# MoonLab-YH/AOD_MEH_HUA

Hardware: AMD Instinct MI355X
Metric: images/sec train+HUA-score, RetinaNet-R50 VOC 512^2 (higher is better)
Workload: dtype bf16x3

## Files before the change

### aod_meh_hua_amd/_C.py

```python
import ctypes as C
import os

import torch

_HERE = os.path.dirname(os.path.abspath(__file__))
LIB_PATH = os.environ.get('AOD_HIP_LIB') or os.path.join(_HERE, 'lib', 'libaodhip.so')


class AodHipError(RuntimeError):
    pass


if not os.path.exists(LIB_PATH):
    raise ImportError(f'{LIB_PATH} is missing: run `python -m aod_meh_hua_amd.build` (hipcc, gfx950). '
                      'There is no CPU fallback for the MEH/HUA hot path.')
lib = C.CDLL(LIB_PATH)


class ConvSeg(C.Structure):
    _fields_ = [('B', C.c_int32), ('H', C.c_int32), ('W', C.c_int32), ('OH', C.c_int32), ('OW', C.c_int32),
                ('src_row0', C.c_int64), ('dst_row0', C.c_int64)]


class ConvDesc(C.Structure):
# ... 77 lines not shown
    'aod_meh_loss_levels_bwd': (C.c_int, [P, P, P, I32, P, P, P, I32, I32, I32, P]),
    'aod_softmax_rowmax': (C.c_int, [P, I32, I64, I32, F32, P, P, I32, P]),
    'aod_topk_stable': (C.c_int, [P, I32, I64, I32, P, I64, P]),
    'aod_pre_nms_levels': (C.c_int, [I32, P, P, P, P, P, P, I32, I32, F32, I32, I32, P, P, P, P, F32, P, P, P, P, P, P, P, I64, P]),
    'aod_gather_decode': (C.c_int, [P, P, P, P, P, I32, I64, I32, I32, I64, P, P, P, P, F32, P, P, P, P, I64, I64, I64, I32, P]),
    'aod_nms_ws_bytes': (SZ, [I32, I32, I32]),
    'aod_multiclass_nms': (C.c_int, [P, P, I32, I32, I32, F32, F32, I32, P, P, P, P, P, P]),
    'aod_hua_ws_bytes': (SZ, [I32, I32]),
    'aod_hua_score': (C.c_int, [P, P, P, P, P, P, P, P, P, I32, I32, I32, I32, I32, F32, F32, F32, I32, U64, P, I32, I32, I32, P, P, I32, P, P, P]),
    'aod_maxpool_fwd': (C.c_int, [P, P, I32, I32, I32, I32, I32, I32, I32, I32, I32, P]),
    'aod_maxpool_bwd': (C.c_int, [P, P, P, I32, I32, I32, I32, I32, I32, I32, I32, I32, P]),
    'aod_l2norm_fwd': (C.c_int, [P, P, P, I64, I32, F32, P]),
    'aod_l2norm_bwd': (C.c_int, [P, P, P, P, P, I64, I32, F32, P]),
    'aod_ssd_loss_fwd': (C.c_int, [P, P, P, P, P, P, I32, I32, I32, I32, I32, F32, P, P, P, P]),
    'aod_ssd_loss_bwd': (C.c_int, [P, P, P, P, P, P, P, P, I32, I32, I32, I32, F32, P, P, P, P, P, P]),
    'aod_synth_normal_images': (C.c_int, [P, I32, I64, U64, P, P]),
    'aod_image_xform': (C.c_int, [P, P, I32, I32, I32, P, P]),
    'aod_x3_split': (C.c_int, [P, P, I64, I32, P]),
    'aod_x3_merge': (C.c_int, [P, P, I64, I32, P]),
    'aod_x3_add': (C.c_int, [P, P, P, I64, P]),
    'aod_x3_nchw_f32_to_s2d': (C.c_int, [P, P, I32, I32, I32, I32, P]),
    'aod_x3_maxpool3x3s2': (C.c_int, [P, P, I32, I32, I32, I32, P]),
    'aod_x3_upsample2x_add_to': (C.c_int, [P, P, P, I32, I32, I32, I32, I32, I32, P]),
    'aod_x3_upsample2x_add_bwd_set': (C.c_int, [P, P, I32, I32, I32, I32, I32, I32, P]),
    'aod_x3_act_bwd': (C.c_int, [P, P, P, P, I64, I32, I32, P]),
    'aod_x3_pad_cast_colsum': (C.c_int, [P, P, P, P, I64, I32, P]),
    'aod_x3_nchw_f32_to_nhwc': (C.c_int, [P, P, I32, I32, I32, I32, P]),
    'aod_x3_maxpool_fwd': (C.c_int, [P, P, I32, I32, I32, I32, I32, I32, I32, I32, I32, P]),
    'aod_x3_maxpool_bwd': (C.c_int, [P, P, P, I32, I32, I32, I32, I32, I32, I32, I32, I32, P]),
    'aod_x3_l2norm_fwd': (C.c_int, [P, P, P, I64, I32, F32, P]),
    'aod_x3_l2norm_bwd': (C.c_int, [P, P, P, P, P, I64, I32, F32, P]),
    'aod_sgd_multi': (C.c_int, [P, P, P, P, I32, F32, P, F32, F32, I32, F32, P]),
    'aod_sgd_multi_clipped': (C.c_int, [P, P, P, P, I32, F32, P, F32, F32, I32, F32, P, P]),
    'aod_grad_norm_multi': (C.c_int, [P, P, I32, F32, F32, I32, P, I64, P, P]),
}
for _n, (_r, _a) in _SIGS.items():
    if hasattr(lib, _n):
        getattr(lib, _n).restype = _r
        getattr(lib, _n).argtypes = _a
lib.aod_last_error.restype = C.c_char_p


def ptr(t):
    if t is None:
        return None
    if not t.is_cuda:
        raise AodHipError('aod_meh_hua_amd ops need tensors on the MI355X (cuda:N); got a CPU tensor. There is no CPU fallback.')
    return C.c_void_p(t.data_ptr())


def stream():
    return C.c_void_p(torch.cuda.current_stream().cuda_stream)


def check(rc, name='aod'):
    if rc != 0:
        raise AodHipError(f'{name} failed ({rc}): {lib.aod_last_error().decode()}')


def call(name, *args):
    check(getattr(lib, name)(*args), name)
```

### aod_meh_hua_amd/csrc/conv.hip

```cpp
#include "common.h"
#include "pointwise.h"
#include "conv_x3p.h"

struct ConvGroup { const bf16_t* x; const bf16_t* w; void* y; const float* pre_shift; const bf16_t* mask; float* colsum; };
struct ConvKParams {
  const bf16_t* x;
  const bf16_t* w;
  void* y;
  const float* pre_scale;
  const float* pre_shift;
  const bf16_t* res;
  const bf16_t* mask;
  const float* post_scale;
  bf16_t* zraw;
  float* colsum;
  int C, N, K, R, S, stride, pad, dil, transposed, relu, out_f32;
  int nseg, M;
  int tiles_m, tiles_n;
  int ksplit;
  float* ws;
  int perm;
  int ngroups;
  ConvGroup grp[4];
  int stagger;
// ... 2093 lines not shown
    __syncthreads();
  }
  if (a.wdot) {
    dot = wave_sum(dot);
    if ((threadIdx.x & 63) == 0) red[threadIdx.x >> 6] = dot;
    __syncthreads();
    if (threadIdx.x == 0) {
      float d = 0.f;
      for (int k = 0; k < UNP_T / 64; ++k) d += red[k];
      a.wdot[oo] = a.bn_s1 ? a.bn_invstd[oo] * (d - a.bn_mean[oo] * a.bn_s1[oo]) : d;
    }
  }
}
__global__ __launch_bounds__(UNP_T) void unpack_wgrad_slabs_kernel(const UnpackArgs a) {
  __shared__ float tile[UNP_CH * 9 + 1];
  __shared__ float red[UNP_T / 64];
  unpack_row(a, blockIdx.x, tile, red);
}
struct UnpackGroups { UnpackArgs g[WG_MAXG]; int blk0[WG_MAXG + 1]; };
__global__ __launch_bounds__(UNP_T) void unpack_wgrad_slabs_grouped_kernel(const UnpackGroups gp) {
  __shared__ float tile[UNP_CH * 9 + 1];
  __shared__ float red[UNP_T / 64];
  const int b = blockIdx.x;
  if (b < gp.blk0[1]) unpack_row(gp.g[0], b, tile, red);
  else if (b < gp.blk0[2]) unpack_row(gp.g[1], b - gp.blk0[1], tile, red);
  else if (b < gp.blk0[3]) unpack_row(gp.g[2], b - gp.blk0[2], tile, red);
  else unpack_row(gp.g[3], b - gp.blk0[3], tile, red);
}
struct PrepItem {
  const float* w; const float* gamma; const float* beta; const float* mean; const float* var;
  bf16_t* wf; bf16_t* wd; float* scale; float* shift; float* invstd;
  int O, I, RS, Ipad, Opad, blk0;
  float eps; int flags;
  long long pad2_[2];
};
constexpr int PREP_T = 32, PREP_RS = 9;
__global__ __launch_bounds__(256) void param_prep_kernel(const PrepItem* __restrict__ items, int nitems) {
  __shared__ float tile[PREP_RS][PREP_T][PREP_T + 1];
  int lo = 0, hi = nitems - 1;
  while (lo < hi) {
    const int mid = (lo + hi + 1) >> 1;
    if (items[mid].blk0 <= (int)blockIdx.x) lo = mid; else hi = mid - 1;
  }
  const PrepItem it = items[lo];
  const int lb = blockIdx.x - it.blk0;
  const int t = threadIdx.x;
  if (it.RS > PREP_RS) {
    const long long nf = (long long)it.O * it.RS * it.Ipad, nd = it.wd ? (long long)it.I * it.RS * it.Opad : 0;
    for (int u = 0; u < 8; ++u) {
      const long long i = (long long)lb * 2048 + u * 256 + t;
      const bool x3 = it.flags & 1;
      if (i < nf) {
        const int cp = i % it.Ipad; const long long r1 = i / it.Ipad; const int rs = r1 % it.RS; const int oo = r1 / it.RS;
        const int c = x3 ? ((cp >> 6) << 5) + (cp & 31) : cp;
        const float v = (c < it.I) ? it.w[((long long)oo * it.I + c) * it.RS + rs] : 0.f;
        const bf16_t h = (bf16_t)v;
        it.wf[i] = (x3 && (cp & 32)) ? (bf16_t)(v - (float)h) : h;
      }
      if (i < nd) {
        const int op = i % it.Opad; const long long r1 = i / it.Opad; const int rs = r1 % it.RS; const int c = r1 / it.RS;
        const int oo = x3 ? ((op >> 6) << 5) + (op & 31) : op;
        float v = 0.f;
        if (oo < it.O) { v = it.w[((long long)oo * it.I + c) * it.RS + rs]; if (it.gamma) v *= it.gamma[oo] * rsqrtf(it.var[oo] + it.eps); }
        const bf16_t h = (bf16_t)v;
        it.wd[i] = (x3 && (op & 32)) ? (bf16_t)(v - (float)h) : h;
      }
      if (it.gamma && i < it.O) {
        const float inv = rsqrtf(it.var[i] + it.eps), sc = it.gamma[i] * inv;
        it.invstd[i] = inv; it.scale[i] = sc; it.shift[i] = it.beta[i] - it.mean[i] * sc;
      }
    }
    return;
  }
  const bool x3 = it.flags & 1;
  const int Il = x3 ? it.Ipad >> 1 : it.Ipad, Ol = x3 ? it.Opad >> 1 : it.Opad;
  const int tiles_c = (Il + PREP_T - 1) / PREP_T;
  const int to = lb / tiles_c, tc = lb - to * tiles_c;
  const int o0 = to * PREP_T, c0 = tc * PREP_T;
  const int RS = it.RS;
  const int run = PREP_T * RS;
  const int pitch = run | 1;
  float* tl = &tile[0][0][0];
  const int cvalid = it.I - c0 < PREP_T ? it.I - c0 : PREP_T;
  {
    const int lim = cvalid * RS;
    const float* src0 = it.w + ((long long)o0 * it.I + c0) * RS;
    const long long ostride = (long long)it.I * RS;
    const bool al = ((((size_t)src0) | ((size_t)ostride * 4)) & 15) == 0;
    f32x4 v[PREP_RS];
    int ol[PREP_RS], idx[PREP_RS];
    const bool full = al && cvalid == PREP_T && o0 + PREP_T <= it.O;
#pragma unroll
    for (int k = 0; k < PREP_RS; ++k) {
      v[k] = (f32x4){0.f, 0.f, 0.f, 0.f};
      if (k < RS) {
        const int e = 4 * (t + k * 256);
        ol[k] = e / run; idx[k] = e - ol[k] * run;
        const float* sp = src0 + ol[k] * ostride + idx[k];
        if (full) v[k] = *reinterpret_cast<const f32x4*>(sp);
        else if (o0 + ol[k] < it.O) {
#pragma unroll
          for (int j = 0; j < 4; ++j) if (idx[k] + j < lim) v[k][j] = sp[j];
        }
      }
    }
#pragma unroll
    for (int k = 0; k < PREP_RS; ++k)
      if (k < RS) {
#pragma unroll
        for (int j = 0; j < 4; ++j) tl[ol[k] * pitch + idx[k] + j] = v[k][j];
      }
  }
  __syncthreads();
  for (int u = t; u < PREP_T * RS * 4; u += 256) {
    const int oct = u & 3, q = u >> 2, ol = q / RS, rs = q - ol * RS;
    const int o = o0 + ol, c = c0 + oct * 8;
    if (o < it.O && c < Il) {
// ... 12 lines not shown
    }
  }
  if (it.wd) {
    __shared__ float s_sc[PREP_T];
    if (t < PREP_T) {
      const int o = o0 + t;
      s_sc[t] = (it.gamma && o < it.O) ? it.gamma[o] * rsqrtf(it.var[o] + it.eps) : 1.f;
    }
    __syncthreads();
    for (int u = t; u < PREP_T * RS * 4; u += 256) {
      const int oct = u & 3, q = u >> 2, cl = q / RS, rs = q - cl * RS;
      const int c = c0 + cl, o = o0 + oct * 8;
      if (c < it.I && o < Ol) {
        bf16x8 v;
#pragma unroll
        for (int j = 0; j < 8; ++j) v[j] = (bf16_t)(tl[(oct * 8 + j) * pitch + cl * RS + rs] * s_sc[oct * 8 + j]);
        if (!x3) *reinterpret_cast<bf16x8*>(it.wd + ((long long)c * RS + rs) * it.Opad + o) = v;
        else {
          bf16x8 l;
#pragma unroll
          for (int j = 0; j < 8; ++j) l[j] = (bf16_t)(tl[(oct * 8 + j) * pitch + cl * RS + rs] * s_sc[oct * 8 + j] - (float)v[j]);
          bf16_t* d = it.wd + ((long long)c * RS + rs) * it.Opad + 2 * o0 + oct * 8;
          *reinterpret_cast<bf16x8*>(d) = v;
          *reinterpret_cast<bf16x8*>(d + 32) = l;
        }
      }
    }
  }
  if (it.gamma && tc == 0 && t < PREP_T && o0 + t < it.O) {
    const int o = o0 + t;
    const float inv = rsqrtf(it.var[o] + it.eps), sc = it.gamma[o] * inv;
    it.invstd[o] = inv; it.scale[o] = sc; it.shift[o] = it.beta[o] - it.mean[o] * sc;
  }
}
extern "C" int aod_param_prep(const void* items_dev, int nitems, int total_blocks, aod_stream_t stream) {
  AOD_CHECK_ARG(items_dev && nitems >= 0 && total_blocks >= 0, "param_prep: bad args");
  if (nitems == 0 || total_blocks == 0) return 0;
  hipLaunchKernelGGL(param_prep_kernel, dim3(total_blocks), dim3(256), 0, (hipStream_t)stream, (const PrepItem*)items_dev, nitems);
  AOD_LAUNCH_CHECK();
  return 0;
}
extern "C" int aod_param_prep_item_bytes(void) { return (int)sizeof(PrepItem); }

static inline int grid_for(long long n) { long long b = (n + 255) / 256; return (int)(b > 4096 ? 4096 : (b < 1 ? 1 : b)); }

extern "C" int aod_pack_weight_fwd(const float* w, void* o, int O, int I, int R, int S, int Ipad, aod_stream_t stream) {
  AOD_CHECK_ARG(w && o && Ipad >= I && Ipad % 8 == 0, "pack_weight_fwd: bad args");
  hipLaunchKernelGGL(pack_w_fwd_kernel, dim3(grid_for((long long)O * R * S * Ipad)), dim3(256), 0, (hipStream_t)stream, w, (bf16_t*)o, O, I, R * S, Ipad);
  AOD_LAUNCH_CHECK();
  return 0;
}
extern "C" int aod_pack_weight_dgrad(const float* w, void* o, int O, int I, int R, int S, int Opad, const float* scale, aod_stream_t stream) {
  AOD_CHECK_ARG(w && o && Opad >= O && Opad % 8 == 0, "pack_weight_dgrad: Opad must be a multiple of 8 and >= O");
  hipLaunchKernelGGL(pack_w_dgrad_kernel, dim3(grid_for((long long)Opad * R * S * I)), dim3(256), 0, (hipStream_t)stream, w, scale, (bf16_t*)o, O, I, R * S, Opad);
  AOD_LAUNCH_CHECK();
  return 0;
}
extern "C" int aod_unpack_wgrad_slabs(const float* dw_slabs, int nslabs, int64_t slab_stride, float* g, int O, int I, int R, int S, int Ipad,
                                      int accumulate, const float* scale, const float* w_oihw, float* wdot, const float* bn_s1,
                                      const float* bn_mean, const float* bn_invstd, aod_stream_t stream) {
  AOD_CHECK_ARG(dw_slabs && g && nslabs >= 1 && slab_stride > 0, "unpack_wgrad_slabs: null / empty");
  AOD_CHECK_ARG(R * S <= 16, "unpack_wgrad_slabs: at most 16 taps (larger filters take aod_unpack_wgrad)");
  AOD_CHECK_ARG(!wdot || w_oihw, "unpack_wgrad_slabs: wdot needs the weights");
  AOD_CHECK_ARG(!bn_s1 || (wdot && bn_mean && bn_invstd), "unpack_wgrad_slabs: BN mode needs wdot, mean and invstd");
  if (O == 0) return 0;
  UnpackArgs a;
// ... 46 lines not shown
```

### aod_meh_hua_amd/functional.py

```python
import torch
from torch.autograd import Function

from . import hipops as ho
from .hipops import Seg


def as_rows(x):
    B, C, H, W = x.shape
    xr = x.permute(0, 2, 3, 1)
    if not xr.is_contiguous():
        xr = xr.contiguous()
    return xr.view(B * H * W, C)


def as_nchw(rows, B, H, W):
    return rows.view(B, H, W, rows.shape[1]).permute(0, 3, 1, 2)


def multi_rows(tensors):
    rows = [as_rows(t) for t in tensors]
    if len(rows) == 1:
        t = tensors[0]
        return rows[0], [Seg(t.shape[0], t.shape[2], t.shape[3], 0)]
    rb = rows[0].shape[1] * rows[0].element_size()
# ... 11 lines not shown


def dense_segs(segs):
    out, r = [], 0
    for s in segs:
        out.append(Seg(s.B, s.H, s.W, r))
        r += s.rows
    return out


import ctypes as _C
import weakref as _weakref


class _PrepRec(_C.Structure):
    _fields_ = [('w', _C.c_void_p), ('gamma', _C.c_void_p), ('beta', _C.c_void_p), ('mean', _C.c_void_p), ('var', _C.c_void_p),
                ('wf', _C.c_void_p), ('wd', _C.c_void_p), ('scale', _C.c_void_p), ('shift', _C.c_void_p), ('invstd', _C.c_void_p),
                ('O', _C.c_int32), ('I', _C.c_int32), ('RS', _C.c_int32), ('Ipad', _C.c_int32), ('Opad', _C.c_int32), ('blk0', _C.c_int32),
                ('eps', _C.c_float), ('pad_', _C.c_int32), ('pad2_', _C.c_int64 * 2)]


class _FragRec(_C.Structure):
    _fields_ = [('src', _C.c_void_p), ('dst', _C.c_void_p), ('rows', _C.c_int32), ('K', _C.c_int32), ('blk0', _C.c_int32), ('pad_', _C.c_int32)]


class _PrepItem:
    __slots__ = ('srcs', 'ver', 'wf', 'wd', 'scale', 'shift', 'invstd', 'eps', 'dims', 'nblk', 'fragf', 'fragd', 'x3')


class ParamPrep:

    def __init__(self):
        self.items, self.order, self.table, self.dirty, self.tables = {}, [], None, True, {}
        self.stems = []

    def watch_stem(self, conv):
        self.stems = [r for r in self.stems if r() is not None and r() is not conv] + [_weakref.ref(conv)]

    def _versions(self, it):
        return tuple(-1 if t is None else t._version for t in (r() if r is not None else None for r in it.srcs))

    def get(self, w, bn, cin_pad, eps):
        it = self.items.get((id(w), ho.X3))
        if it is not None and it.srcs[0]() is not w:
            it = None
        if it is None:
            it = self._register(w, bn, cin_pad, eps)
        if it.ver != self._versions(it):
            self.refresh()
        return it

    def _register(self, w, bn, cin_pad, eps):
        O, I, R, S = w.shape
        dev = w.device
        it = _PrepItem()
        it.srcs = [_weakref.ref(w)] + [(_weakref.ref(t) if t is not None else None) for t in (bn if bn is not None else (None,) * 4)]
        it.x3 = ho.X3
        if it.x3:
            assert cin_pad == ho.xw(I), f'x3: input rows of {cin_pad} columns for a filter with {I} input channels'
            opad = ho.xw(O)
            it.wf = torch.empty(O, R, S, cin_pad, dtype=torch.bfloat16, device=dev)
            it.wd = torch.empty(I, R, S, opad, dtype=torch.bfloat16, device=dev) if I % 32 == 0 else None
        else:
            opad = (O + 7) // 8 * 8
            it.wf = torch.empty(O, R, S, cin_pad, dtype=torch.bfloat16, device=dev)
            it.wd = torch.empty(I, R, S, opad, dtype=torch.bfloat16, device=dev) if cin_pad == I else None
        if bn is not None:
            it.scale, it.shift, it.invstd = (torch.empty(O, dtype=torch.float32, device=dev) for _ in range(3))
        else:
            it.scale = it.shift = it.invstd = None
        it.eps, it.dims, it.ver = float(eps), (O, I, R * S, cin_pad, opad), None
        it.fragf = it.fragd = None
        if R * S <= 9 and it.x3:
            it.nblk = (opad // 64) * (cin_pad // 64)
        elif R * S <= 9:
            it.nblk = ((opad + 31) // 32) * ((cin_pad + 31) // 32)
        else:
            it.nblk = (max(O * R * S * cin_pad, I * R * S * opad if it.wd is not None else 0, O) + 2047) // 2048
        self.items[(id(w), it.x3)] = it
        self.dirty = True
        return it

    def frag(self, it, which):
        name = 'fragf' if which == 'f' else 'fragd'
        t = getattr(it, name)
        if t is None:
            src = it.wf if which == 'f' else it.wd
            rows = src.shape[0]
            assert rows % 256 == 0 and (src.numel() // rows) % 64 == 0, 'frag images need rows % 256 == 0 and K % 64 == 0'
            t = torch.empty(src.numel(), dtype=torch.bfloat16, device=src.device)
            setattr(it, name, t)
            self.tables, it.ver = {}, None
            self.refresh()
        return t

    def refresh_if_stale(self):
        for r in self.stems:
            conv = r()
            if conv is not None and not torch.cuda.is_current_stream_capturing():
                _stem_w4(conv)
        if any(it.x3 == ho.X3 and it.ver != self._versions(it) for it in self.items.values()):
            self.refresh()

    def refresh(self):
        assert not torch.cuda.is_current_stream_capturing(), \
            'parameter preparation inside a HIP-graph capture: call PREP.refresh_if_stale() before capturing / replaying'
        dead = [k for k, it in self.items.items() if it.srcs[0]() is None or any(r is not None and r() is None for r in it.srcs[1:])]
        for k in dead:
            del self.items[k]
            self.dirty = True
        if self.dirty:
            self.order = list(self.items.values())
            self.tables = {}
            self.dirty = False
        stale = tuple(i for i, it in enumerate(self.order) if it.x3 == ho.X3 and it.ver != self._versions(it))
        if not stale:
            return
        ent = self.tables.get(stale)
        if ent is None:
            if len(self.tables) > 16:
                self.tables.clear()
            recs = (_PrepRec * len(stale))()
            blk = 0
            for r, i in zip(recs, stale):
                it = self.order[i]
                src = [x() if x is not None else None for x in it.srcs]
                for t in src:
                    assert t is None or (t.dtype == torch.float32 and t.is_contiguous()), 'parameters must be contiguous fp32'
                r.w, r.gamma, r.beta, r.mean, r.var = (None if t is None else t.data_ptr() for t in src)
                r.wf, r.wd = it.wf.data_ptr(), (it.wd.data_ptr() if it.wd is not None else None)
                r.scale, r.shift, r.invstd = ((t.data_ptr() if t is not None else None) for t in (it.scale, it.shift, it.invstd))
                r.O, r.I, r.RS, r.Ipad, r.Opad = it.dims
                r.blk0, r.eps, r.pad_ = blk, it.eps, int(it.x3)
                blk += it.nblk
            host = torch.frombuffer(bytearray(bytes(recs)), dtype=torch.uint8)
            dev = self.order[stale[0]].wf.device
            fl = [(src, dst) for i in stale for src, dst in ((self.order[i].wf, self.order[i].fragf), (self.order[i].wd, self.order[i].fragd))
                  if dst is not None]
            ftab, fblk = None, 0
            if fl:
                frecs = (_FragRec * len(fl))()
                for r, (src, dst) in zip(frecs, fl):
                    r.src, r.dst, r.rows, r.K, r.blk0 = src.data_ptr(), dst.data_ptr(), src.shape[0], src.numel() // src.shape[0], fblk
                    fblk += (src.numel() + 2047) // 2048
                ftab = torch.frombuffer(bytearray(bytes(frecs)), dtype=torch.uint8).to(dev)
            ent = self.tables[stale] = (host.to(dev), blk, ftab, len(fl), fblk)
        self.table = ent[0]
        ho.call('aod_param_prep', ho.ptr(ent[0]), len(stale), ent[1], ho.stream())
        if ent[2] is not None:
            ho.call('aod_frag_pack', ho.ptr(ent[2]), ent[3], ent[4], ho.stream())
        for i in stale:
            self.order[i].ver = self._versions(self.order[i])


PREP = ParamPrep()


import os as _os
_FUSE_ACT = _os.environ.get('AOD_FUSE_ACT', '1') != '0'


_PREC = _os.environ.get('AOD_CONV_PREC', 'bf16x3')
assert _PREC in ('bf16', 'bf16x3'), f'AOD_CONV_PREC={_PREC!r}: bf16x3 (reference precision) or bf16 (fast mode)'
ho.X3 = _PREC == 'bf16x3'


def set_precision(p):
    global _PREC
    assert p in ('bf16', 'bf16x3')
    _PREC = p
    ho.X3 = p == 'bf16x3'


def x3_to_f32(x, channels=None):
    if not ho.X3 or x.dtype != torch.bfloat16:
        return x.float()
    B, Wd, H, W = x.shape
    rows = ho.x3_merge(as_rows(x), channels)
    return as_nchw(rows, B, H, W)


class ForkFn(Function):

    @staticmethod
    def forward(ctx, x, n):
        return tuple(x.view_as(x) for _ in range(n))

    @staticmethod
    def backward(ctx, *gs):
        tot = None
        for g in gs:
            if g is None:
                continue
            g = g.contiguous(memory_format=torch.channels_last)
            tot = g if tot is None else as_nchw(ho.x3_add(as_rows(tot), as_rows(g)), g.shape[0], g.shape[2], g.shape[3])
        return tot, None


def fork(x, n):
    if not ho.X3 or n == 1 or not (torch.is_grad_enabled() and x.requires_grad):
        return [x] * n
    return list(ForkFn.apply(x, n))


def get_precision():
    return _PREC


def mode_key():
    return (_PREC, bool(ho.DETERMINISTIC))


class ActSlot:
    __slots__ = ('masked', 's1', 'res_ok', 'res_grad')

    def __init__(self):
        self.masked, self.s1 = False, None
        self.res_ok, self.res_grad = False, None


class BwdChain:
    __slots__ = ('meta', 'x_rows', 'prep', 'out')

    def __init__(self):
        self.meta, self.x_rows, self.prep, self.out = {}, {}, {}, {}


def bwd_chain_for(blk, x):
    on = _os.environ.get('AOD_FUSE_BOTTLENECK_BWD', '1') != '0' and not ho.DETERMINISTIC
    if ho.X3 and _os.environ.get('AOD_FUSE_BOTTLENECK128_X3_BWD', '1') == '0':
        return None
    return BwdChain() if on and _FUSE_ACT and bottleneck128_train_applies(blk, x) else None


def set_deterministic(on=True):
    ho.set_deterministic(on)


class GradAcc:
    __slots__ = ('n', 'arrived', 'partial', 'slot', '__weakref__')

    def __init__(self, slot=None):
        self.n, self.arrived, self.partial = 0, 0, None
# ... 940 lines not shown
```

### aod_meh_hua_amd/graphs.py

```python
import torch

from . import functional as AF
from . import hipops as ho
from .datasets import DeviceImageBatch

torch.autograd.graph.set_warn_on_accumulate_grad_stream_mismatch(False)
from .models.dense_heads.L_anchor_head import PackedGT


def _pin_caches():
    from . import scoring
    return (dict(ho._ROW_TABLES), dict(ho._DW), dict(ho._SLABS), list(AF.PREP.items.values()), AF.PREP.table, dict(scoring._META))


def _low_memory(dev, frac=0.25):
    try:
        free, total = torch.cuda.mem_get_info(dev)
        return free < frac * total
    except Exception:
        return False


def _unwrap(model):
    return model.module if hasattr(model, 'module') else model


def _plain(data, dev):
    from .mmcv_lite import DataContainer

    def un(x):
        if isinstance(x, DataContainer):
            d = x.data
            return d[0] if isinstance(d, list) and len(d) == 1 else d
        return x
    return {k: un(v) for k, v in data.items()}


class GraphedTrainStep:
    MAX_GRAPHS = 16

    def __init__(self, model, optimizer, optimizer_L, grad_sync=None, gmax=64, warmup=2, **step_kwargs):
        self.model, self.module = model, _unwrap(model)
        self.opt, self.opt_L, self.sync = optimizer, optimizer_L, grad_sync
        self.gmax, self.warmup, self.kw = gmax, warmup, step_kwargs
        self.cache = {}
# ... 175 lines not shown
        self._load(d)
        self.opt.device_lr(), self.opt_L.device_lr()
        self.module.train()
        snap = self._snapshot()
        side = torch.cuda.Stream()
        side.wait_stream(torch.cuda.current_stream())
        with torch.cuda.stream(side):
            for _ in range(self.warmup):
                self._run_eager(comm=False)
        torch.cuda.current_stream().wait_stream(side)
        torch.cuda.synchronize()
        ho.reset_zero_arena()
        AF.PREP.refresh_if_stale()
        segs = self._segments(dist_mode)
        graphs = []
        if not dist_mode:
            g = torch.cuda.CUDAGraph()
            with torch.cuda.graph(g, capture_error_mode='thread_local'):
                for _, f in segs:
                    f()
            graphs.append(g)
        else:
            pool = torch.cuda.graph_pool_handle()
            for tag, f in segs:
                g = torch.cuda.CUDAGraph()
                with torch.cuda.graph(g, pool=pool, capture_error_mode='thread_local'):
                    f()
                graphs.append(g)
                self._between(tag, capturing=True)
            self.cur['tags'] = [tag for tag, _ in segs]
        ho.reset_zero_arena()
        self._restore(snap)
        AF.PREP.refresh_if_stale()
        self.cur.update(graphs=graphs, keep=_pin_caches(), touched=self._params(self.opt) + self._params(self.opt_L))
        return self.cur

    def maybe(self, data_batch):
        d = _plain(data_batch, self.dev)
        sig = self._signature(d)
        want = self._known(sig) or sig[0] == (self.last_sig or (None,))[0]
        self.last_sig = sig
        if not want:
            return None
        return self(data_batch)

    def __call__(self, data_batch):
        d = _plain(data_batch, self.dev)
        sig = self._signature(d)
        ent = self._lookup(sig)
        if ent is None:
            while self.cache and (len(self.cache) >= self.MAX_GRAPHS or _low_memory(self.dev)):
                self.cache.pop(next(iter(self.cache)))
                import gc
                gc.collect()
                torch.cuda.empty_cache()
            ent = self._build(d)
        self.cache[sig] = self.cur = ent
        if not ent.pop('loaded', False):
            self._load(d)
        self.opt.device_lr(), self.opt_L.device_lr()
        AF.PREP.refresh_if_stale()
        self.inflight = []
        for i, g in enumerate(ent['graphs']):
            g.replay()
            if len(ent['graphs']) > 1:
                self._between(ent['tags'][i])
        tp = [p for p in ent['touched'] if p.grad is not None]
        torch._C._autograd._unsafe_set_version_counter(tp, [p._version + 1 for p in tp])
        out, loss_L = ent['live'][0], ent['live_L']
        pa, pb = self.cur['pack'].clone(), self.cur['pack_L'].clone()
        log_vars = type(out['log_vars'])(zip(out['log_vars'].keys(), pa[1:].unbind(0)))
        log_vars.update(zip(loss_L['log_vars'].keys(), pb.unbind(0)))
        return dict(loss=pa[0], log_vars=log_vars, num_samples=out['num_samples'])


class GraphedScore:
    MAX_GRAPHS = 16

    def __init__(self, model, warmup=2, pipeline=None, **score_kwargs):
        import os
        import weakref
        self._model = weakref.ref(_unwrap(model))
        self.kw, self.warmup = score_kwargs, warmup
        self.cache, self.pending = {}, None
        self.dev = next(_unwrap(model).parameters()).device
        m = _unwrap(model)
        two_phase = (hasattr(m, 'extract_feat') and hasattr(getattr(m, 'bbox_head', None), 'test_heads') and not score_kwargs.get('isEval')
                     and getattr(m.test_cfg, 'uncertainty_pool', None) in ('Entropy_NMS', 'Entropy_ALL'))
        self.pipe = two_phase and (os.environ.get('AOD_SCORE_PIPELINE', '1') != '0' if pipeline is None else bool(pipeline))
        self.s_conv = self.s_tail = None

    @property
    def module(self):
        m = self._model()
        if m is None:
            raise RuntimeError('GraphedScore outlived its model')
        return m

    def _run(self, sl):
        from . import scoring
        with torch.no_grad(), scoring.static_meta(sl['hw'], sl['sc']):
# ... 146 lines not shown
```

### aod_meh_hua_amd/optim.py

```python
import ctypes as C

import torch

from ._C import call, stream


class FusedSGD(torch.optim.Optimizer):

    def __init__(self, params, lr=1e-3, momentum=0.0, dampening=0, weight_decay=0.0, nesterov=False, grad_clip=None, skip_nonfinite=False):
        assert dampening == 0 and not nesterov, 'the AL configs use plain momentum SGD'
        if grad_clip is not None:
            grad_clip = dict(grad_clip)
            if 'max_norm' not in grad_clip:
                raise ValueError(f'grad_clip needs max_norm: {grad_clip}')
            if float(grad_clip.get('norm_type', 2)) != 2.0:
                raise ValueError(f'grad_clip norm_type={grad_clip["norm_type"]!r}: only the 2-norm is implemented')
            if not float(grad_clip['max_norm']) > 0:
                raise ValueError(f'grad_clip max_norm must be positive: {grad_clip["max_norm"]!r}')
        super().__init__(params, dict(lr=lr, momentum=momentum, weight_decay=weight_decay))
        self.grad_scale = 1.0
        self._lr_dev = {}
        self.grad_clip, self.skip_nonfinite = grad_clip, bool(skip_nonfinite)
        self._clip_state, self._clip_ws, self._clip_keep = None, None, []

    def _clip_buffers(self, ntensors, dev):
        need = 96 * max(int(ntensors), 1)
        if self._clip_state is None or self._clip_ws.numel() < need:
            if torch.cuda.is_current_stream_capturing():
                raise RuntimeError('FusedSGD(grad_clip=...): call device_lr() (or run one eager step) before capturing step() in a graph')
            if self._clip_state is None:
                self._clip_state = torch.zeros(4, dtype=torch.float32, device=dev)
            if self._clip_ws is not None:
                self._clip_keep.append(self._clip_ws)
            self._clip_ws = torch.empty(need, dtype=torch.float32, device=dev)

    def clip_state(self):
        return self._clip_state if self.grad_clip is not None else None

    def device_lr(self):
        for gi, group in enumerate(self.param_groups):
            ent = self._lr_dev.get(gi)
            if ent is None:
                dev = group['params'][0].device
                self._lr_dev[gi] = [torch.full((1,), float(group['lr']), dtype=torch.float32, device=dev), float(group['lr'])]
            elif ent[1] != float(group['lr']):
                ent[0].fill_(float(group['lr']))
                ent[1] = float(group['lr'])
        if self.grad_clip is not None:
            params = [p for g in self.param_groups for p in g['params']]
            if params:
                self._clip_buffers(len(params), params[0].device)

    @torch.no_grad()
    def step(self, closure=None):
        if self._lr_dev and not torch.cuda.is_current_stream_capturing():
            self.device_lr()
        from . import functional as _AF
        _AF._WgradQueue.flush()
        touched, keep = [], []
        batches = []
        for gi, group in enumerate(self.param_groups):
            ps, gs, ms, ns, first = [], [], [], [], None
            for p in group['params']:
                if p.grad is None:
                    continue
                assert p.dtype == torch.float32 and p.is_contiguous()
                g = p.grad if p.grad.is_contiguous() else p.grad.contiguous()
                keep.append(g)
                st = self.state[p]
                is_first = 'momentum_buffer' not in st
                if is_first:
                    st['momentum_buffer'] = torch.empty_like(p)
                if first is None:
                    first = is_first
                if is_first != first:
                    batches.append((gi, group, first, ps, gs, ms, ns))
                    ps, gs, ms, ns, first = [], [], [], [], is_first
                ps.append(p.data_ptr()), gs.append(g.data_ptr()), ms.append(st['momentum_buffer'].data_ptr()), ns.append(p.numel())
                touched.append(p)
            batches.append((gi, group, first, ps, gs, ms, ns))
        coef = None
        if self.grad_clip is not None and touched:
            coef = self._grad_norm([g for b in batches for g in b[4]], [n for b in batches for n in b[6]], touched[0].device)
        for gi, group, first, ps, gs, ms, ns in batches:
            self._gi = gi
            self._launch(ps, gs, ms, ns, group, first, coef)
        if touched:
            torch._C._autograd._unsafe_set_version_counter(touched, [p._version + 1 for p in touched])

    def _grad_norm(self, gs, ns, dev):
        n = len(gs)
        self._clip_buffers(n, dev)
        from .hipops import prof_bytes
        prof_bytes('grad_norm_multi', sum(ns) * 4,
                   lambda: call('aod_grad_norm_multi', (C.c_void_p * n)(*gs), (C.c_int64 * n)(*ns), n, float(self.grad_scale),
                                float(self.grad_clip['max_norm']), int(self.skip_nonfinite), C.c_void_p(self._clip_ws.data_ptr()),
                                self._clip_ws.numel(), C.c_void_p(self._clip_state.data_ptr()), stream()))
        return C.c_void_p(self._clip_state.data_ptr() + 4)

    def _launch(self, ps, gs, ms, ns, group, first, coef=None):
        n = len(ps)
        if n == 0:
            return
        arr = C.c_void_p * n
        ent = self._lr_dev.get(self._gi)
        from .hipops import prof_bytes
        args = (arr(*ps), arr(*gs), arr(*ms), (C.c_int64 * n)(*ns), n, float(group['lr']),
                C.c_void_p(ent[0].data_ptr()) if ent is not None else None, float(group['momentum']),
                float(group['weight_decay']), int(bool(first)), float(self.grad_scale))
        if coef is None:
            prof_bytes('sgd_multi', sum(ns) * (16 if first else 20), lambda: call('aod_sgd_multi', *args, stream()))
        else:
            prof_bytes('sgd_multi', sum(ns) * (16 if first else 20), lambda: call('aod_sgd_multi_clipped', *args, coef, stream()))


def build_optimizer(model, cfg, grad_clip=None, skip_nonfinite=False):
    cfg = dict(cfg)
    t = cfg.pop('type')
    assert t == 'SGD', 'the AL configs use SGD'
    cfg.pop('paramwise_cfg', None)
    module = model.module if hasattr(model, 'module') else model
    return FusedSGD([p for p in module.parameters() if p.requires_grad], grad_clip=grad_clip, skip_nonfinite=skip_nonfinite, **cfg)
```

### include/aod_hip.h

```cpp
#ifndef AOD_HIP_H
#define AOD_HIP_H
#include <stddef.h>
#include <stdint.h>

#ifdef __cplusplus
extern "C" {
#endif

typedef void* aod_stream_t;

const char* aod_last_error(void);
int aod_version(void);

typedef struct {
  int32_t B, H, W;
  int32_t OH, OW;
  int64_t src_row0;
  int64_t dst_row0;
} aod_conv_seg_t;

typedef struct {
  int32_t C, N;
  int32_t R, S;
  int32_t stride, pad, dil;
// ... 63 lines not shown

int aod_conv2d_grouped(const aod_conv_desc_t* desc, int ngroups, const void* const* src, const void* const* w_packed, void* const* dst,
                       const float* const* pre_shift, const void* const* mask, float* const* colsum, aod_stream_t stream);

int aod_conv2d_wgrad(const aod_conv_desc_t* desc, const void* x, const void* dz, float* dw_f32,
                     const void* row_table, aod_stream_t stream);
int aod_conv2d_wgrad_splits(const aod_conv_desc_t* desc);
int aod_conv2d_wgrad_slabs(const aod_conv_desc_t* desc, const void* x, const void* dz, float* slabs, int nslabs, int64_t slab_stride,
                           const void* row_table, aod_stream_t stream);
int aod_conv2d_wgrad_group_plan(const aod_conv_desc_t* const* descs, int n, int32_t* splits_out);
int aod_conv2d_wgrad_grouped(const aod_conv_desc_t* const* descs, int n, const void* const* x, const void* const* dz, float* const* slabs,
                             const int32_t* nslabs, const int64_t* slab_stride, const void* const* row_table, aod_stream_t stream);
size_t aod_conv_row_table_bytes(const aod_conv_desc_t* desc);
int aod_conv_row_table(const aod_conv_desc_t* desc, void* table, aod_stream_t stream);

int aod_pack_weight_fwd(const float* w_oihw, void* w_packed, int O, int I, int R, int S, int Ipad, aod_stream_t stream);
int aod_pack_weight_dgrad(const float* w_oihw, void* w_packed, int O, int I, int R, int S, int Opad, const float* scale,
                          aod_stream_t stream);
int aod_unpack_wgrad(float* dw_orsi, float* grad_oihw, int O, int I, int R, int S, int Ipad, int accumulate, int clear_src,
                     const float* scale, const float* w_oihw, float* wdot, const float* bn_s1, const float* bn_mean,
                     const float* bn_invstd, aod_stream_t stream);

int aod_unpack_wgrad_slabs(const float* dw_slabs, int nslabs, int64_t slab_stride, float* grad_oihw, int O, int I, int R, int S, int Ipad,
                           int accumulate, const float* scale, const float* w_oihw, float* wdot, const float* bn_s1,
                           const float* bn_mean, const float* bn_invstd, aod_stream_t stream);

int aod_unpack_wgrad_slabs_grouped(int n, const float* const* dw_slabs, const int32_t* nslabs, const int64_t* slab_stride, float* const* g,
                                   const int32_t* O, const int32_t* I, const int32_t* R, const int32_t* S, const int32_t* Ipad,
                                   const int32_t* accumulate, const float* const* scale, const float* const* w_oihw, float* const* wdot,
                                   const float* const* bn_s1, const float* const* bn_mean, const float* const* bn_invstd,
                                   aod_stream_t stream);
int aod_param_prep(const void* items_dev, int nitems, int total_blocks, aod_stream_t stream);
int aod_param_prep_item_bytes(void);

int aod_nchw_f32_to_nhwc_bf16(const float* src, void* dst, int B, int C, int H, int W, int Cpad, aod_stream_t stream);
int aod_nchw_f32_to_s2d_bf16(const float* src, void* dst, int B, int C, int H, int W, aod_stream_t stream);
int aod_stem_pool_fwd(const void* x_s2d, const void* w_packed, const float* scale, const float* shift, void* y, int B, int H2, int W2,
                      aod_stream_t stream);
int aod_maxpool3x3s2(const void* src, void* dst, int B, int H, int W, int C, aod_stream_t stream);
int aod_upsample2x_add(const void* src, void* dst, int B, int h, int w, int C, int H, int W, aod_stream_t stream);
int aod_upsample2x_add_bwd(const void* g_dst, void* g_src_accum, int B, int h, int w, int C, int H, int W, aod_stream_t stream);
int aod_upsample2x_add_to(const void* top, const void* lateral, void* out, int B, int h, int w, int C, int H, int W, aod_stream_t stream);
int aod_upsample2x_add_bwd_set(const void* g_dst, void* g_src, int B, int h, int w, int C, int H, int W, aod_stream_t stream);
int aod_act_bwd(const void* g, const void* a, const void* z, const float* scale, const float* mean, const float* invstd,
                void* dz, void* gmask_out, float* dbeta, float* dgamma, int64_t M, int N, int relu, int g_is_f32,
                aod_stream_t stream);
int aod_pad_cast_colsum(const void* g, const float* relu_out_f32, void* dz, float* colsum, int64_t M, int N, int Npad,
                        int g_is_f32, aod_stream_t stream);
int aod_add_relu(const void* a, const void* b, void* out, int64_t n, aod_stream_t stream);

int aod_halo_conv3x3_applies(const aod_conv_desc_t* desc);
int aod_halo_conv3x3(const aod_conv_desc_t* desc, const void* src, const void* w_packed, void* dst, const float* pre_shift,
                     const void* mask, float* colsum, aod_stream_t stream);

size_t aod_loss_partials_len(int64_t nrows);
int aod_edl_focal_l1_fwd(const float* cls, const int64_t* labels, const float* label_w,
                         const float* bbox_pred, const float* bbox_tgt, const float* bbox_w,
                         int64_t nrows, int C, float gamma, float alpha,
                         float* loss_noR, float* sums3, float* partials, aod_stream_t stream);
int aod_edl_focal_l1_bwd(const float* cls, const int64_t* labels, const float* label_w,
                         const float* bbox_pred, const float* bbox_tgt, const float* bbox_w,
                         int64_t nrows, int C, float gamma, float alpha,
                         const float* g_cls, const float* g_bbox, const float* g_noR, float g_noR_scalar, int g_noR_is_scalar,
                         void* grad_cls, void* grad_bbox, int out_bf16, int A, int pitch_cls, int pitch_box,
                         aod_stream_t stream);
int aod_edl_focal_elem(const float* cls, const int64_t* labels, int64_t nrows, int C, float gamma, float alpha,
// ... 135 lines not shown
```

Before: 644.2.

## Fuse SGD momentum update into conv weight pack/param-prep kernel

Adds an sgd_prep kernel that performs the SGD momentum update for conv weights (RS<=9) and immediately writes the packed bf16x3 forward/dgrad weights from the updated values held in registers and shared memory. The optimizer routes fusable parameters to this path and marks their prep entries fresh, so the separate param_prep pass on the next forward is skipped. This removes one full read of fp32 weights and an extra kernel pass per step. In exchange the optimizer, prep cache and graph replay become coupled, and there is more bookkeeping around table validity and the grad-clip coefficient.

Measured after the change: 642.0. Within noise of the previous version (-0.3%).

```diff
diff --git a/aod_meh_hua_amd/_C.py b/aod_meh_hua_amd/_C.py
--- a/aod_meh_hua_amd/_C.py
+++ b/aod_meh_hua_amd/_C.py
@@ -133,6 +133,7 @@
     'aod_x3_l2norm_bwd': (C.c_int, [P, P, P, P, P, I64, I32, F32, P]),
     'aod_sgd_multi': (C.c_int, [P, P, P, P, I32, F32, P, F32, F32, I32, F32, P]),
     'aod_sgd_multi_clipped': (C.c_int, [P, P, P, P, I32, F32, P, F32, F32, I32, F32, P, P]),
+    'aod_sgd_prep': (C.c_int, [P, I32, P, P, F32, P, F32, F32, I32, F32, P, P]),
     'aod_grad_norm_multi': (C.c_int, [P, P, I32, F32, F32, I32, P, I64, P, P]),
 }
 for _n, (_r, _a) in _SIGS.items():
diff --git a/aod_meh_hua_amd/csrc/conv.hip b/aod_meh_hua_amd/csrc/conv.hip
--- a/aod_meh_hua_amd/csrc/conv.hip
+++ b/aod_meh_hua_amd/csrc/conv.hip
@@ -2149,20 +2149,28 @@
   bf16_t* wf; bf16_t* wd; float* scale; float* shift; float* invstd;
   int O, I, RS, Ipad, Opad, blk0;
   float eps; int flags;
-  long long pad2_[2];
+  float* mom; long long pad2_;
+};
+constexpr int SGDP_MAX = 48;
+struct SgdPrepArgs {
+  const float* g[SGDP_MAX];
+  int blk_base;
+  float lr; const float* lr_dev; float momentum, decay; int first_step; float grad_scale; const float* coef_dev;
 };
 constexpr int PREP_T = 32, PREP_RS = 9;
-__global__ __launch_bounds__(256) void param_prep_kernel(const PrepItem* __restrict__ items, int nitems) {
+template <bool SGD>
+__device__ __forceinline__ void param_prep_body(const PrepItem* __restrict__ items, int nitems, const int blk, const SgdPrepArgs* __restrict__ sa) {
   __shared__ float tile[PREP_RS][PREP_T][PREP_T + 1];
   int lo = 0, hi = nitems - 1;
   while (lo < hi) {
     const int mid = (lo + hi + 1) >> 1;
-    if (items[mid].blk0 <= (int)blockIdx.x) lo = mid; else hi = mid - 1;
+    if (items[mid].blk0 <= blk) lo = mid; else hi = mid - 1;
   }
   const PrepItem it = items[lo];
-  const int lb = blockIdx.x - it.blk0;
+  const int lb = blk - it.blk0;
   const int t = threadIdx.x;
   if (it.RS > PREP_RS) {
+    if constexpr (SGD) return;
     const long long nf = (long long)it.O * it.RS * it.Ipad, nd = it.wd ? (long long)it.I * it.RS * it.Opad : 0;
     for (int u = 0; u < 8; ++u) {
       const long long i = (long long)lb * 2048 + u * 256 + t;
@@ -2199,7 +2207,68 @@
   const int pitch = run | 1;
   float* tl = &tile[0][0][0];
   const int cvalid = it.I - c0 < PREP_T ? it.I - c0 : PREP_T;
-  {
+  if constexpr (SGD) {
+    const float lr = sa->lr_dev ? *sa->lr_dev : sa->lr;
+    const float coef = sa->coef_dev ? *sa->coef_dev : 1.0f;
+    const bool skip = coef < 0.f;
+    const float grad_scale = sa->grad_scale * coef;
+    const float momentum = sa->momentum, decay = sa->decay;
+    const bool first = sa->first_step != 0;
+    const int lim = cvalid * RS;
+    const long long off0 = ((long long)o0 * it.I + c0) * RS, ostride = (long long)it.I * RS;
+    float* wp = const_cast<float*>(it.w) + off0;
+    const float* gp = sa->g[lo] + off0;
+    float* mp = it.mom + off0;
+    const bool full = cvalid == PREP_T && o0 + PREP_T <= it.O && ((((size_t)wp) | ((size_t)gp) | ((size_t)mp) | ((size_t)ostride * 4)) & 15) == 0;
+    for (int k0 = 0; k0 < RS; k0 += 3) {
+      f32x4 pv[3], gv[3], mv[3];
+      int ol[3], idx[3];
+#pragma unroll
+      for (int kk = 0; kk < 3; ++kk) {
+        pv[kk] = gv[kk] = mv[kk] = (f32x4){0.f, 0.f, 0.f, 0.f};
+        ol[kk] = idx[kk] = 0;
+        if (k0 + kk < RS) {
+          const int e = 4 * (t + (k0 + kk) * 256);
+          ol[kk] = e / run; idx[kk] = e - ol[kk] * run;
+          const long long off = ol[kk] * ostride + idx[kk];
+          if (full) {
+            pv[kk] = *reinterpret_cast<const f32x4*>(wp + off); gv[kk] = *reinterpret_cast<const f32x4*>(gp + off);
+            if (!first) mv[kk] = *reinterpret_cast<const f32x4*>(mp + off);
+          } else if (o0 + ol[kk] < it.O) {
+#pragma unroll
+            for (int j = 0; j < 4; ++j)
+              if (idx[kk] + j < lim) { pv[kk][j] = wp[off + j]; gv[kk][j] = gp[off + j]; if (!first) mv[kk][j] = mp[off + j]; }
+          }
+        }
+      }
+#pragma unroll
+      for (int kk = 0; kk < 3; ++kk)
+        if (k0 + kk < RS) {
+          const long long off = ol[kk] * ostride + idx[kk];
+          const bool row = full || o0 + ol[kk] < it.O;
+          f32x4 po = pv[kk];
+          if (!skip) {
+#pragma unroll
+            for (int u = 0; u < 4; ++u) {
+              const float d = gv[kk][u] * grad_scale + decay * pv[kk][u];
+              const float b = first ? d : momentum * mv[kk][u] + d;
+              mv[kk][u] = b;
+              po[u] = pv[kk][u] - lr * b;
+            }
+            if (full) {
+              *reinterpret_cast<f32x4*>(mp + off) = mv[kk];
+              *reinterpret_cast<f32x4*>(wp + off) = po;
+            } else if (row) {
+#pragma unroll
+              for (int j = 0; j < 4; ++j)
+                if (idx[kk] + j < lim) { mp[off + j] = mv[kk][j]; wp[off + j] = po[j]; }
+            }
+          }
+#pragma unroll
+          for (int j = 0; j < 4; ++j) tl[ol[kk] * pitch + idx[kk] + j] = (full || (row && idx[kk] + j < lim)) ? po[j] : 0.f;
+        }
+    }
+  } else {
     const int lim = cvalid * RS;
     const float* src0 = it.w + ((long long)o0 * it.I + c0) * RS;
     const long long ostride = (long long)it.I * RS;
@@ -2278,6 +2347,33 @@
     const float inv = rsqrtf(it.var[o] + it.eps), sc = it.gamma[o] * inv;
     it.invstd[o] = inv; it.scale[o] = sc; it.shift[o] = it.beta[o] - it.mean[o] * sc;
   }
+}
+__global__ __launch_bounds__(256) void param_prep_kernel(const PrepItem* __restrict__ items, int nitems) {
+  param_prep_body<false>(items, nitems, (int)blockIdx.x, nullptr);
+}
+__global__ __launch_bounds__(256) void sgd_prep_kernel(const PrepItem* __restrict__ items, int nitems, const SgdPrepArgs sa) {
+  param_prep_body<true>(items, nitems, (int)blockIdx.x + sa.blk_base, &sa);
+}
+extern "C" int aod_sgd_prep(const void* items_dev, int nitems, const int32_t* blk0_host, void* const* grads, float lr, const float* lr_dev,
+                            float momentum, float weight_decay, int first_step, float grad_scale, const float* coef_dev, aod_stream_t stream) {
+  AOD_CHECK_ARG(nitems >= 0 && (nitems == 0 || (items_dev && blk0_host && grads)), "sgd_prep: bad args");
+  for (int s0 = 0; s0 < nitems; s0 += SGDP_MAX) {
+    const int cnt = nitems - s0 < SGDP_MAX ? nitems - s0 : SGDP_MAX;
+    SgdPrepArgs sa;
+    for (int i = 0; i < SGDP_MAX; ++i) sa.g[i] = i < cnt ? (const float*)grads[s0 + i] : nullptr;
+    for (int i = 0; i < cnt; ++i) {
+      AOD_CHECK_ARG(sa.g[i], "sgd_prep: null gradient pointer");
+      AOD_CHECK_ARG(blk0_host[s0 + i + 1] >= blk0_host[s0 + i], "sgd_prep: block offsets must not decrease");
+    }
+    sa.blk_base = blk0_host[s0];
+    sa.lr = lr; sa.lr_dev = lr_dev; sa.momentum = momentum; sa.decay = weight_decay; sa.first_step = first_step; sa.grad_scale = grad_scale;
+    sa.coef_dev = coef_dev;
+    const int blocks = blk0_host[s0 + cnt] - blk0_host[s0];
+    if (blocks == 0) continue;
+    hipLaunchKernelGGL(sgd_prep_kernel, dim3(blocks), dim3(256), 0, (hipStream_t)stream, (const PrepItem*)items_dev + s0, cnt, sa);
+    AOD_LAUNCH_CHECK();
+  }
+  return 0;
 }
 extern "C" int aod_param_prep(const void* items_dev, int nitems, int total_blocks, aod_stream_t stream) {
   AOD_CHECK_ARG(items_dev && nitems >= 0 && total_blocks >= 0, "param_prep: bad args");
diff --git a/aod_meh_hua_amd/functional.py b/aod_meh_hua_amd/functional.py
--- a/aod_meh_hua_amd/functional.py
+++ b/aod_meh_hua_amd/functional.py
@@ -67,6 +67,7 @@
 
     def __init__(self):
         self.items, self.order, self.table, self.dirty, self.tables = {}, [], None, True, {}
+        self.sgd_tables = {}
         self.stems = []
 
     def watch_stem(self, conv):
@@ -129,6 +130,61 @@
             self.refresh()
         return t
 
+    def _fill_rec(self, r, it, blk):
+        src = [x() if x is not None else None for x in it.srcs]
+        for t in src:
+            assert t is None or (t.dtype == torch.float32 and t.is_contiguous()), 'parameters must be contiguous fp32'
+        r.w, r.gamma, r.beta, r.mean, r.var = (None if t is None else t.data_ptr() for t in src)
+        r.wf, r.wd = it.wf.data_ptr(), (it.wd.data_ptr() if it.wd is not None else None)
+        r.scale, r.shift, r.invstd = ((t.data_ptr() if t is not None else None) for t in (it.scale, it.shift, it.invstd))
+        r.O, r.I, r.RS, r.Ipad, r.Opad = it.dims
+        r.blk0, r.eps, r.pad_ = blk, it.eps, int(it.x3)
+
+    @staticmethod
+    def _frag_table(its, dev):
+        fl = [(src, dst) for it in its for src, dst in ((it.wf, it.fragf), (it.wd, it.fragd)) if dst is not None]
+        if not fl:
+            return None, 0, 0
+        frecs, fblk = (_FragRec * len(fl))(), 0
+        for r, (src, dst) in zip(frecs, fl):
+            r.src, r.dst, r.rows, r.K, r.blk0 = src.data_ptr(), dst.data_ptr(), src.shape[0], src.numel() // src.shape[0], fblk
+            fblk += (src.numel() + 2047) // 2048
+        return torch.frombuffer(bytearray(bytes(frecs)), dtype=torch.uint8).to(dev), len(fl), fblk
+
+    def fusable(self, p):
+        it = self.items.get((id(p), ho.X3))
+        if it is None or it.srcs[0]() is not p or it.dims[2] > 9 or any(r is not None and r() is None for r in it.srcs[1:]):
+            return None
+        return it
+
+    def sgd_table(self, its, moms):
+        key = tuple((it.srcs[0]().data_ptr(), m.data_ptr(), it.wf.data_ptr(), it.wd.data_ptr() if it.wd is not None else 0,
+                     it.fragf.data_ptr() if it.fragf is not None else 0, it.fragd.data_ptr() if it.fragd is not None else 0)
+                    for it, m in zip(its, moms))
+        ent = self.sgd_tables.get(key)
+        if ent is None:
+            if torch.cuda.is_current_stream_capturing():
+                return None
+            if len(self.sgd_tables) > 16:
+                self.sgd_tables.clear()
+            recs, blk0 = (_PrepRec * len(its))(), (_C.c_int32 * (len(its) + 1))()
+            blk = 0
+            for i, (r, it, m) in enumerate(zip(recs, its, moms)):
+                assert m.dtype == torch.float32 and m.is_contiguous() and m.numel() == it.srcs[0]().numel()
+                self._fill_rec(r, it, blk)
+                r.pad2_[0] = m.data_ptr()
+                blk0[i] = blk
+                blk += it.nblk
+            blk0[len(its)] = blk
+            dev = its[0].wf.device
+            ent = self.sgd_tables[key] = (torch.frombuffer(bytearray(bytes(recs)), dtype=torch.uint8).to(dev), blk0,
+                                          *self._frag_table(its, dev), list(its), list(moms))
+        return ent
+
+    def mark_fresh(self, its):
+        for it in its:
+            it.ver = self._versions(it)
+
     def refresh_if_stale(self):
         for r in self.stems:
             conv = r()
@@ -158,28 +214,11 @@
             recs = (_PrepRec * len(stale))()
             blk = 0
             for r, i in zip(recs, stale):
-                it = self.order[i]
-                src = [x() if x is not None else None for x in it.srcs]
-                for t in src:
-                    assert t is None or (t.dtype == torch.float32 and t.is_contiguous()), 'parameters must be contiguous fp32'
-                r.w, r.gamma, r.beta, r.mean, r.var = (None if t is None else t.data_ptr() for t in src)
-                r.wf, r.wd = it.wf.data_ptr(), (it.wd.data_ptr() if it.wd is not None else None)
-                r.scale, r.shift, r.invstd = ((t.data_ptr() if t is not None else None) for t in (it.scale, it.shift, it.invstd))
-                r.O, r.I, r.RS, r.Ipad, r.Opad = it.dims
-                r.blk0, r.eps, r.pad_ = blk, it.eps, int(it.x3)
-                blk += it.nblk
+                self._fill_rec(r, self.order[i], blk)
+                blk += self.order[i].nblk
             host = torch.frombuffer(bytearray(bytes(recs)), dtype=torch.uint8)
             dev = self.order[stale[0]].wf.device
-            fl = [(src, dst) for i in stale for src, dst in ((self.order[i].wf, self.order[i].fragf), (self.order[i].wd, self.order[i].fragd))
-                  if dst is not None]
-            ftab, fblk = None, 0
-            if fl:
-                frecs = (_FragRec * len(fl))()
-                for r, (src, dst) in zip(frecs, fl):
-                    r.src, r.dst, r.rows, r.K, r.blk0 = src.data_ptr(), dst.data_ptr(), src.shape[0], src.numel() // src.shape[0], fblk
-                    fblk += (src.numel() + 2047) // 2048
-                ftab = torch.frombuffer(bytearray(bytes(frecs)), dtype=torch.uint8).to(dev)
-            ent = self.tables[stale] = (host.to(dev), blk, ftab, len(fl), fblk)
+            ent = self.tables[stale] = (host.to(dev), blk, *self._frag_table([self.order[i] for i in stale], dev))
         self.table = ent[0]
         ho.call('aod_param_prep', ho.ptr(ent[0]), len(stale), ent[1], ho.stream())
         if ent[2] is not None:
@@ -193,6 +232,16 @@
 
 import os as _os
 _FUSE_ACT = _os.environ.get('AOD_FUSE_ACT', '1') != '0'
+_STEP_FUSE = _os.environ.get('AOD_STEP_FUSE', '1') != '0'
+
+
+def set_step_fusion(on):
+    global _STEP_FUSE
+    _STEP_FUSE = bool(on)
+
+
+def step_fusion():
+    return _STEP_FUSE
 
 
 _PREC = _os.environ.get('AOD_CONV_PREC', 'bf16x3')
@@ -243,7 +292,7 @@
 
 
 def mode_key():
-    return (_PREC, bool(ho.DETERMINISTIC))
+    return (_PREC, bool(ho.DETERMINISTIC), _STEP_FUSE)
 
 
 class ActSlot:
diff --git a/aod_meh_hua_amd/graphs.py b/aod_meh_hua_amd/graphs.py
--- a/aod_meh_hua_amd/graphs.py
+++ b/aod_meh_hua_amd/graphs.py
@@ -10,7 +10,8 @@
 
 def _pin_caches():
     from . import scoring
-    return (dict(ho._ROW_TABLES), dict(ho._DW), dict(ho._SLABS), list(AF.PREP.items.values()), AF.PREP.table, dict(scoring._META))
+    return (dict(ho._ROW_TABLES), dict(ho._DW), dict(ho._SLABS), list(AF.PREP.items.values()), AF.PREP.table, dict(AF.PREP.sgd_tables),
+            dict(scoring._META))
 
 
 def _low_memory(dev, frac=0.25):
@@ -252,7 +253,8 @@
         ho.reset_zero_arena()
         self._restore(snap)
         AF.PREP.refresh_if_stale()
-        self.cur.update(graphs=graphs, keep=_pin_caches(), touched=self._params(self.opt) + self._params(self.opt_L))
+        fused = [(it, it.fragf, it.fragd) for o in (self.opt, self.opt_L) if hasattr(o, 'fused_items') for it in o.fused_items()]
+        self.cur.update(graphs=graphs, keep=_pin_caches(), touched=self._params(self.opt) + self._params(self.opt_L), fused=fused)
         return self.cur
 
     def maybe(self, data_batch):
@@ -287,6 +289,7 @@
                 self._between(ent['tags'][i])
         tp = [p for p in ent['touched'] if p.grad is not None]
         torch._C._autograd._unsafe_set_version_counter(tp, [p._version + 1 for p in tp])
+        AF.PREP.mark_fresh([it for it, ff, fd in ent['fused'] if it.fragf is ff and it.fragd is fd])
         out, loss_L = ent['live'][0], ent['live_L']
         pa, pb = self.cur['pack'].clone(), self.cur['pack_L'].clone()
         log_vars = type(out['log_vars'])(zip(out['log_vars'].keys(), pa[1:].unbind(0)))
diff --git a/aod_meh_hua_amd/optim.py b/aod_meh_hua_amd/optim.py
--- a/aod_meh_hua_amd/optim.py
+++ b/aod_meh_hua_amd/optim.py
@@ -22,6 +22,7 @@
         self._lr_dev = {}
         self.grad_clip, self.skip_nonfinite = grad_clip, bool(skip_nonfinite)
         self._clip_state, self._clip_ws, self._clip_keep = None, None, []
+        self._fused = []
 
     def _clip_buffers(self, ntensors, dev):
         need = 96 * max(int(ntensors), 1)
@@ -59,6 +60,9 @@
         _AF._WgradQueue.flush()
         touched, keep = [], []
         batches = []
+        prep = _AF.PREP if _AF.step_fusion() else None
+        fbatches = {}
+        norm_gs, norm_ns = [], []
         for gi, group in enumerate(self.param_groups):
             ps, gs, ms, ns, first = [], [], [], [], None
             for p in group['params']:
@@ -71,6 +75,13 @@
                 is_first = 'momentum_buffer' not in st
                 if is_first:
                     st['momentum_buffer'] = torch.empty_like(p)
+                norm_gs.append(g.data_ptr()), norm_ns.append(p.numel())
+                it = prep.fusable(p) if prep is not None else None
+                if it is not None:
+                    fb = fbatches.setdefault((gi, is_first), [[], [], []])
+                    fb[0].append(it), fb[1].append(g.data_ptr()), fb[2].append(st['momentum_buffer'])
+                    touched.append(p)
+                    continue
                 if first is None:
                     first = is_first
                 if is_first != first:
@@ -79,14 +90,30 @@
                 ps.append(p.data_ptr()), gs.append(g.data_ptr()), ms.append(st['momentum_buffer'].data_ptr()), ns.append(p.numel())
                 touched.append(p)
             batches.append((gi, group, first, ps, gs, ms, ns))
+        tables = {k: prep.sgd_table(fb[0], fb[2]) for k, fb in fbatches.items()}
+        for k, fb in fbatches.items():
+            if tables[k] is None:
+                batches.append((k[0], self.param_groups[k[0]], k[1], [it.srcs[0]().data_ptr() for it in fb[0]], fb[1],
+                                [m.data_ptr() for m in fb[2]], [m.numel() for m in fb[2]]))
         coef = None
         if self.grad_clip is not None and touched:
-            coef = self._grad_norm([g for b in batches for g in b[4]], [n for b in batches for n in b[6]], touched[0].device)
+            coef = self._grad_norm(norm_gs, norm_ns, touched[0].device)
         for gi, group, first, ps, gs, ms, ns in batches:
             self._gi = gi
             self._launch(ps, gs, ms, ns, group, first, coef)
+        self._fused = []
+        for (gi, first), fb in fbatches.items():
+            if tables[(gi, first)] is not None:
+                self._gi = gi
+                self._launch_prep(tables[(gi, first)], fb, self.param_groups[gi], first, coef)
+                self._fused += fb[0]
         if touched:
             torch._C._autograd._unsafe_set_version_counter(touched, [p._version + 1 for p in touched])
+        if self._fused and not torch.cuda.is_current_stream_capturing():
+            _AF.PREP.mark_fresh(self._fused)
+
+    def fused_items(self):
+        return list(self._fused)
 
     def _grad_norm(self, gs, ns, dev):
         n = len(gs)
@@ -113,6 +140,18 @@
         else:
             prof_bytes('sgd_multi', sum(ns) * (16 if first else 20), lambda: call('aod_sgd_multi_clipped', *args, coef, stream()))
 
+    def _launch_prep(self, table, fb, group, first, coef=None):
+        tab, blk0, ftab, nfrag, fblk = table[:5]
+        n = len(fb[0])
+        ent = self._lr_dev.get(self._gi)
+        from .hipops import prof_bytes
+        prof_bytes('sgd_prep', sum(m.numel() for m in fb[2]) * (24 if first else 28),
+                   lambda: call('aod_sgd_prep', C.c_void_p(tab.data_ptr()), n, blk0, (C.c_void_p * n)(*fb[1]), float(group['lr']),
+                                C.c_void_p(ent[0].data_ptr()) if ent is not None else None, float(group['momentum']),
+                                float(group['weight_decay']), int(bool(first)), float(self.grad_scale), coef, stream()))
+        if ftab is not None:
+            call('aod_frag_pack', C.c_void_p(ftab.data_ptr()), nfrag, fblk, stream())
+
 
 def build_optimizer(model, cfg, grad_clip=None, skip_nonfinite=False):
     cfg = dict(cfg)
diff --git a/include/aod_hip.h b/include/aod_hip.h
--- a/include/aod_hip.h
+++ b/include/aod_hip.h
@@ -119,6 +119,8 @@
                                    aod_stream_t stream);
 int aod_param_prep(const void* items_dev, int nitems, int total_blocks, aod_stream_t stream);
 int aod_param_prep_item_bytes(void);
+int aod_sgd_prep(const void* items_dev, int nitems, const int32_t* blk0_host, void* const* grads, float lr, const float* lr_dev,
+                 float momentum, float weight_decay, int first_step, float grad_scale, const float* coef_dev, aod_stream_t stream);
 
 int aod_nchw_f32_to_nhwc_bf16(const float* src, void* dst, int B, int C, int H, int W, int Cpad, aod_stream_t stream);
 int aod_nchw_f32_to_s2d_bf16(const float* src, void* dst, int B, int C, int H, int W, aod_stream_t stream);
```
